# kursawe/OpticalFlow

Hardware: AMD Instinct MI355X
Metric: frame-pairs/sec (higher is better)
Workload: dtype f64; 1 GPU; 1024x1024x256 synthetic translating texture (seed 1), speed_alpha=1, remodelling_alpha=1e4, rtol=1e-06, all 255 pairs solved to the stopping rule; frames_per_gpu=256, pairs_in_flight=255, levels=9, coarse_stencils=float8, vcycle_vectors=coarse_float32, w_cycle_level=1, w_cycle_visits=3, warm_start_stride=3, allgather=False, gather_chunks=1, converged=True

## Files before the change

### opticalflow_amd/csrc/vof.hip

```cpp
#include "vof_device.hpp"
#include "vof_sweep0r.hpp"
#include "vof_sweep0p.hpp"
#include "vof_stream0.hpp"
#include "vof_direct.hpp"
#include "vof_boxflow.hpp"
#include "vof_boxsweep.hpp"
#include "vof_blursweep.hpp"
#include "vof_compare.hpp"
#include "vof_liushen.hpp"
#include "../../include/vof.h"

#include <fcntl.h>
#include <unistd.h>

#include <algorithm>
#include <atomic>
#include <chrono>
#include <cmath>
#include <condition_variable>
#include <cstdio>
#include <cstdlib>
#include <cstring>
#include <mutex>
#include <string>
// ... 60 lines not shown
    int nd = 0;
    int* h_active = nullptr;
    int* h_alist = nullptr;
    PairScalars* h_sc = nullptr;
    double* h_func3 = nullptr;
    char* h_bounce = nullptr;
    hipEvent_t ev_batch[2] = {nullptr, nullptr};
    double* st_movie = nullptr;
    double* st_out[4] = {nullptr, nullptr, nullptr, nullptr};
    double* st_out2[4] = {nullptr, nullptr, nullptr, nullptr};
    hipStream_t copy_stream = nullptr;
    hipEvent_t ev_solved[2] = {nullptr, nullptr}, ev_copied[2] = {nullptr, nullptr}, ev_uploaded[2] = {nullptr, nullptr};
    double* st_movie2 = nullptr;
    double *blur_tmp = nullptr, *blur_w = nullptr, *blur_io = nullptr;
    double* bf_scratch = nullptr;
    double* sw_scratch = nullptr;
    size_t sw_planes = 0;
    bool sw_by_budget = false;
    char* sw_aux = nullptr;
    size_t sw_aux_bytes = 0;
    bool bf_lds_set = false;
    bool bl_lds_set = false;
    bool ls_lds_set = false;
    double* tex_tab = nullptr;
    size_t tex_cap = 0;
    double* gm_V = nullptr;
    GmresState* gm_state = nullptr;
    double* gm_partials = nullptr;
    int* gm_cycle = nullptr;
    int gm_m = 0;
    long long gmres_pairs = 0;
    struct Alloc { void* raw; char* user; size_t bytes; const char* name; int line; };
    std::vector<Alloc> allocs;
    int c_bytes_per_point = 0;
    size_t bytes = 0;
    std::string err;
    const double* frames = nullptr;
    int npairs = 0;
    vof_params prm;
    int cfmt = 0;
    bool fused = true;
    bool fold_stored = false;
    bool fuse_revisit = true;
    bool direct_on = false;
    int dir_cap = 0;
    double *dir_T = nullptr, *dir_tabs = nullptr, *dir_W = nullptr, *dir_r = nullptr, *dir_y = nullptr, *dir_x = nullptr, *dir_t = nullptr;
    int *dir_ipiv = nullptr, *dir_info = nullptr;
    double *dir_R = nullptr, *dir_C = nullptr, *dir_D = nullptr;
    int dir_ld = 0;
    long long direct_pairs = 0;
    bool fuse_rr = true;
    bool fuse_b = true;
    int fused_ends = 3;
    long sweep0r_min_blocks = 512;
    int tail_first = -1;
    size_t tail_lds = 0;
    TailArgs tail;
    int tail_key[6] = {-9, -9, -9, -9, -9, -9};
    bool prof = false;
    int prof_kid = -1, prof_level = -1;
    std::vector<ProfRec> recs;
    std::vector<hipEvent_t> free_events;
    long long prof_dropped = 0;
    double prof_ms[VOF_K_COUNT][16];
    long long prof_n[VOF_K_COUNT][16];
    long long prof_units[VOF_K_COUNT][16];
    double prof_bytes[VOF_K_COUNT][16];
    double prof_moved[VOF_K_COUNT][16];
    int cur_units = 0;
    int dbg_sync = 0;
    long long dbg_seq = 0;
    std::string dbg_fault;
    int dbg_fd = -1;
    bool dbg_canary = false;
    bool dbg_alloc_log = false;
    bool dbg_poison = false;
    size_t part_per_pair = 0;
    vof_ctx* lane_parent = nullptr;
    int lane_lo = 0, lane_slots = 0;
    int dir_ok = -1;
    hipStream_t lane_stream[MAX_LANES] = {};
    hipEvent_t lane_ev[MAX_LANES][2] = {};
    hipEvent_t ev_fork = nullptr;
    hipEvent_t group_ev[MAX_LANES * MAX_LANE_GROUPS] = {};
};

static std::string g_create_error;

namespace {

void dbg_sync_check(vof_ctx* c, const char* what, int level) {
    if (!c->dbg_sync) return;
    ++c->dbg_seq;
    char line[256];
    if (c->dbg_fd >= 0) {
        int n = snprintf(line, sizeof line, "in flight: scope #%lld '%s' level %d, %d pairs, grid %dx%d (%d levels)%-40s\n", c->dbg_seq, what, level,
                         c->cur_units, c->Ni, c->Nj, (int)c->L.size(), "");
        if (pwrite(c->dbg_fd, line, (size_t)n, 0) < 0) {  }
    }
    hipError_t e = hipStreamSynchronize(c->stream);
    hipError_t e2 = hipGetLastError();
    if (e == hipSuccess) e = e2;
    if (e != hipSuccess && c->dbg_fault.empty()) {
        snprintf(line, sizeof line, "VOF_DEBUG_SYNC: scope #%lld, kernel class '%s', level %d, %d pairs, image %dx%d: %s", c->dbg_seq, what, level,
                 c->cur_units, c->Ni, c->Nj, hipGetErrorString(e));
        c->dbg_fault = line;
// ... 602 lines not shown
           s0r_row<2, true, false, 0, float, 1, 0, float>(c, p, f0, nslots, a) || s0r_row<2, true, false, 0, double, 1, 0, float>(c, p, f0, nslots, a) ||
           shapes(IntTag<2>{}, IntTag<0>{}) || shapes(IntTag<2>{}, IntTag<1>{}) || shapes(IntTag<1>{}, IntTag<0>{}) || shapes(IntTag<1>{}, IntTag<1>{});
}

template <int NS, bool EC, bool FZ, int TR, typename ET = double>
bool s0m_row(vof_ctx* c, const L0Pass& p, const Fine0& f0, int nslots, const L0Ptrs& a) {
    if (p.NS != NS || p.EC != EC || p.FROM_ZERO != FZ || p.TRAIL != TR || p.ET32 != is_f32<ET>()) return false;
    k_sweep0m<NS, EC, FZ, TR, ET><<<dim3(p.blocks * nslots), p.block, p.lds, c->stream>>>(
        f0, c->L[0].ni, c->L[0].nj, p.TI, p.PO, p.nx, p.ny, nslots, (const double*)a.x_in, (double*)a.x_out, (const double*)a.b, a.active,
        (const ET*)a.ecoarse, p.nci, p.ncj, a.tr);
    return true;
}
bool launch_s0m(vof_ctx* c, const L0Pass& p, const Fine0& f0, int nslots, const L0Ptrs& a) {
    auto shapes = [&](auto ns) {
        constexpr int NS = decltype(ns)::value;
        return s0m_row<NS, true, false, 1, float>(c, p, f0, nslots, a) || s0m_row<NS, true, false, 0, float>(c, p, f0, nslots, a) ||
               s0m_row<NS, true, false, 1>(c, p, f0, nslots, a) || s0m_row<NS, false, false, 1>(c, p, f0, nslots, a) ||
               s0m_row<NS, true, false, 0>(c, p, f0, nslots, a) || s0m_row<NS, false, true, 0>(c, p, f0, nslots, a) ||
               s0m_row<NS, false, false, 0>(c, p, f0, nslots, a);
    };
    return shapes(IntTag<2>{}) || shapes(IntTag<1>{});
}

template <int NS, bool EC, bool FZ, int PO>
bool s0p_row(vof_ctx* c, const L0Pass& p, const Fine0& f0, int nslots, const L0Ptrs& a) {
    if (p.NS != NS || p.EC != EC || p.FROM_ZERO != FZ || p.PO != PO) return false;
    k_sweep0p<NS, EC, FZ, PO><<<dim3(p.blocks * nslots), p.block, p.lds, c->stream>>>(
        f0, c->L[0].ni, c->L[0].nj, p.TI, p.nx, p.nxp, p.ny, nslots, (const float*)a.x_in, (float*)a.x_out, (const float*)a.b, a.active,
        (const float*)a.ecoarse, p.nci, p.ncj);
    return true;
}
bool launch_s0p(vof_ctx* c, const L0Pass& p, const Fine0& f0, int nslots, const L0Ptrs& a) {
    auto shapes = [&](auto ns, auto po) {
        constexpr int NS = decltype(ns)::value, PO = decltype(po)::value;
        return s0p_row<NS, true, false, PO>(c, p, f0, nslots, a) || s0p_row<NS, false, true, PO>(c, p, f0, nslots, a) ||
               s0p_row<NS, false, false, PO>(c, p, f0, nslots, a);
    };
    return shapes(IntTag<2>{}, IntTag<0>{}) || shapes(IntTag<2>{}, IntTag<1>{}) || shapes(IntTag<1>{}, IntTag<0>{}) || shapes(IntTag<1>{}, IntTag<1>{});
}

template <typename VT, bool EC, bool FZ>
bool s0_row(vof_ctx* c, const L0Pass& p, const Fine0& f0, int nslots, const L0Ptrs& a) {
    if (p.EC != EC || p.FROM_ZERO != FZ) return false;
    k_sweep0<VT, EC, FZ><<<dim3(p.blocks * nslots), p.block, p.lds, c->stream>>>(
        f0, c->L[0].ni, c->L[0].nj, p.TI, p.PO, p.nx, p.ny, nslots, (const VT*)a.x_in, (VT*)a.x_out, (const VT*)a.b, a.active,
        (const VT*)a.ecoarse, p.nci, p.ncj);
    return true;
}
template <typename VT>
bool launch_s0(vof_ctx* c, const L0Pass& p, const Fine0& f0, int nslots, const L0Ptrs& a) {
    return s0_row<VT, true, false>(c, p, f0, nslots, a) || s0_row<VT, false, true>(c, p, f0, nslots, a) || s0_row<VT, false, false>(c, p, f0, nslots, a);
}

void fold_s_epilogue(vof_ctx* c, int np, const L0Pass& p) {
    const size_t len = 3 * c->L[0].npts;
    { Prof pr(c, VOF_K_VECTOR, 0); k_scalar<S_S><<<np, 64, 0, c->stream>>>(c->sc, c->partials, (int)p.blocks, c->active, c->prm.rtol, c->prm.max_iterations); }
    { Prof pr(c, VOF_K_VECTOR, 0);
      if (p.XT32) k_fix_half<float><<<dim3(64, np), RBLK, 0, c->stream>>>(c->kx, (const float*)c->ky, len, c->sc);
      else k_fix_half<double><<<dim3(64, np), RBLK, 0, c->stream>>>(c->kx, (const double*)c->ky, len, c->sc);
      k_clear_half<<<(np + 255) / 256, 256, 0, c->stream>>>(c->sc, np); }
}

template <typename VT>
struct SmoothArgs {
    bool from_zero = false;
    bool reverse = false;
    const VT* ecoarse = nullptr;
    bool ec32 = false;
    bool allow_swap = false;
    bool final_smooth = false;
    bool out64 = false;
    bool skip0 = false;
    void* rr_out = nullptr;
    bool rr_f32 = false;
    int nsweeps = 1;
    bool trail = false;
};

template <typename VT>
void sweep_level_t(vof_ctx* c, int l, const VT* x_in, VT* x_out, const VT* b, int np, ActiveSet active, const SmoothArgs<VT>& a,
                   CycleIO& io) {
    Level& lv = c->L[l];
    const VT* ecoarse = a.ecoarse;
    const int po = a.reverse ? 1 : 0;
    if (l == 0 && lv.C == nullptr) {
        L0Req rq;
        rq.from_zero = x_in == nullptr; rq.po = po; rq.nsweeps = a.nsweeps;
        rq.ec = ecoarse != nullptr; rq.ec32 = a.ec32;
        rq.trail = a.trail && io.trail.v != nullptr; rq.trail_dot = io.trail.dotvec != nullptr;
        rq.rr = a.rr_out != nullptr; rq.rr_f32 = a.rr_f32;
        rq.bf = io.bf_done ? 0 : io.bf_mode;
        rq.x32 = c->h32;
        const L0Pass p = plan_l0_pass<VT>(c, rq);
        if (p.XT32 != c->h32) { c->err = "float32 level-0 hand-off: the planned pass does not store float32"; io.failed = true; return; }
        const S0Trail no_trail{nullptr, nullptr, 0, nullptr};
        const L0Ptrs ptrs{x_in, x_out, b, active, ecoarse,
                          p.rr() ? S0Trail{(double*)a.rr_out, nullptr, 0, nullptr} : (p.trail() ? io.trail : no_trail),
                          p.bf() ? io.bf : S0BSrc{nullptr, nullptr, nullptr, nullptr, nullptr, nullptr}};
        const Fine0 f0{c->frames, frame_stride(c), c->Nj, c->prm.speed_alpha, c->prm.remodelling_alpha, c->prm.reference_quirks, c->pp};
        bool launched = false;
        {
            Prof pr(c, VOF_K_GS0, 0, p.algo, p.moved);
            const int nslots = pair_slots(c, active, np);
            switch (p.fam) {
                case L0_SWEEP0R: launched = launch_s0r(c, p, f0, nslots, ptrs); break;
                case L0_SWEEP0M: launched = launch_s0m(c, p, f0, nslots, ptrs); break;
                case L0_SWEEP0P: launched = launch_s0p(c, p, f0, nslots, ptrs); break;
                case L0_SWEEP0: launched = launch_s0<VT>(c, p, f0, nslots, ptrs); break;
            }
        }
        if (!launched) { c->err = "internal: the library holds no kernel for the planned level-0 pass"; io.failed = true; return; }
        if (p.trail()) io.trail_nblk = (int)p.blocks;
        if (p.rr()) io.rr_done = true;
// ... 540 lines not shown
    for (int p = 0; p < ni; ++p) {
        if (trace && (p < 2 || p == ni - 1)) { HIPCHK(hipStreamSynchronize(s)); fprintf(stderr, "[vof] direct_setup: row %d of %d (m = %d, %d pairs)\n", p, ni, m, np); fflush(stderr); }
        double* Tp = c->dir_T + (size_t)p * ld * ld;
        if (p > 0) k_dir_W<<<gm, 256, 0, s>>>(Tp - (size_t)ld * ld, sT, c->dir_tabs + (size_t)(p - 1) * rowTab, sTab, nj, c->dir_W, sW, ld);
        k_dir_schur<<<gs, 256, 0, s>>>(c->dir_tabs + (size_t)p * rowTab, sTab, nj, p > 0 ? c->dir_W : nullptr, sW, Tp, sT, ld);
        if (blocked) {
            for (int kt = 0; kt < nt; ++kt) {
                k_dir_bgj_panel<<<dim3(nt, 2, np), 256, bgj_lds, s>>>(Tp, sT, ld, kt, c->dir_R, c->dir_C, c->dir_D, c->dir_info);
                k_dir_bgj_update<<<dim3(nt, nt, np), 256, bgj_lds, s>>>(Tp, sT, ld, kt, c->dir_R, c->dir_C, c->dir_D);
            }
        } else {
            k_dir_invert<<<np, 1024, 2 * (size_t)m * sizeof(double), s>>>(Tp, sT, m, c->dir_ipiv, c->dir_info);
        }
    }
    HIPCHK(hipGetLastError());
    std::vector<int> info((size_t)np);
    HIPCHK(hipMemcpyAsync(info.data(), c->dir_info, (size_t)np * sizeof(int), hipMemcpyDeviceToHost, s));
    HIPCHK(hipStreamSynchronize(s));
    for (int k = 0; k < np; ++k)
        if (info[k] != 0) { c->err = "direct preconditioner: a Schur block of pair " + std::to_string(k) + " of the batch is singular"; return -2; }
    return 0;
}

template <typename VT>
int direct_apply_t(vof_ctx* c, VT* z, const VT* r, int np) {
    const int ni = c->L[0].ni, nj = c->L[0].nj, m = 3 * nj, ld = c->dir_ld;
    const size_t sT = (size_t)ni * ld * ld, sTab = (size_t)ni * nj * DIR_TAB, rowTab = (size_t)nj * DIR_TAB, sV = (size_t)ni * m;
    hipStream_t s = c->stream;
    Prof pr(c, VOF_K_COARSE_SOLVE, 0);
    const dim3 gp(64, np), gv((m + 255) / 256, np), gg((m + 63) / 64, np);
    k_dir_permute<const VT, true><<<gp, 256, 0, s>>>(r, c->dir_r, ni, nj);
    for (int p = 0; p < ni; ++p) {
        if (p > 0) k_dir_gemv<<<gg, 256, 0, s>>>(c->dir_T + (size_t)(p - 1) * ld * ld, sT, m, c->dir_y + (size_t)(p - 1) * m, sV, c->dir_t, (size_t)m, ld);
        k_dir_rowupdate<<<gv, 256, 0, s>>>(c->dir_tabs + (size_t)p * rowTab, sTab, nj, -1, c->dir_r + (size_t)p * m, sV,
                                          p > 0 ? c->dir_t : nullptr, (size_t)m, c->dir_y + (size_t)p * m, sV);
    }
    for (int p = ni - 1; p >= 0; --p) {
        k_dir_rowupdate<<<gv, 256, 0, s>>>(c->dir_tabs + (size_t)p * rowTab, sTab, nj, +1, c->dir_y + (size_t)p * m, sV,
                                          p + 1 < ni ? c->dir_x + (size_t)(p + 1) * m : nullptr, sV, c->dir_t, (size_t)m);
        k_dir_gemv<<<gg, 256, 0, s>>>(c->dir_T + (size_t)p * ld * ld, sT, m, c->dir_t, (size_t)m, c->dir_x + (size_t)p * m, sV, ld);
    }
    k_dir_permute<VT, false><<<gp, 256, 0, s>>>(z, c->dir_x, ni, nj);
    return 0;
}

struct BatchReq {
    const double* frames;
    int np;
    const PairParam* table;
    const int* guess;
    bool direct;
    double *vx, *vy, *gm, *speed;
    vof_pair_stats* stats;
};

int solve_batch(vof_ctx* c, const BatchReq& rq) {
    const vof_params& P = c->prm;
    const double* const frames_dev = rq.frames;
    const int np = rq.np;
    vof_pair_stats* const stats = rq.stats;
    struct ReqGuard { vof_ctx* c; ~ReqGuard() { c->pp = nullptr; c->direct_on = false; } } req_guard{c};
    const int* guess_src = nullptr;
    if (rq.table || rq.guess) {
        if (rq.table && !c->pp_buf) { if (int rc = dev_alloc(c, &c->pp_buf, (size_t)c->B)) return rc; }
        if (rq.guess && !c->warm_src) { if (int rc = dev_alloc(c, &c->warm_src, (size_t)c->B)) return rc; }
        HIPCHK(hipStreamSynchronize(c->stream));
        if (rq.table) {
            HIPCHK(hipMemcpyAsync(c->pp_buf, rq.table, (size_t)np * sizeof(PairParam), hipMemcpyHostToDevice, c->stream));
            c->pp = c->pp_buf;
        }
        if (rq.guess) {
            HIPCHK(hipMemcpyAsync(c->warm_src, rq.guess, (size_t)np * sizeof(int), hipMemcpyHostToDevice, c->stream));
            guess_src = c->warm_src;
        }
    }
    c->direct_on = rq.direct;
    struct MaxItGuard { vof_params& p; int saved; ~MaxItGuard() { p.max_iterations = saved; } } max_it_guard{c->prm, c->prm.max_iterations};
    constexpr int MG_ATTEMPT_CAP = 150;
    if (P.preconditioner == 2 && !c->direct_on && c->L.size() > 1 && P.max_iterations > MG_ATTEMPT_CAP && 3 * c->L[0].nj <= 3100 &&
        direct_ok_for_fallback(c))
        c->prm.max_iterations = MG_ATTEMPT_CAP;
    if (stats) HIPCHK(hipEventRecord(c->ev_batch[0], c->stream));
    c->vfloat = (P.vcycle_precision == 1 || P.vcycle_precision == 2) && c->fused && c->L.size() > 1 && !c->direct_on;
    c->vcoarse32 = P.vcycle_precision == 3 && !c->direct_on;
    c->h32 = false;
    if (c->direct_on) {
        if (np > c->dir_cap) { c->err = "batch larger than the direct preconditioner's buffers"; return -1; }
        c->frames = frames_dev;
        c->npairs = np;
        c->cur_units = np;
        if (int rc = direct_setup(c, np)) return rc;
        c->direct_pairs += np;
    } else if (int rc = setup_batch(c, frames_dev, np)) return rc;
    Level& f = c->L[0];
    const size_t len = 3 * f.npts;
    hipStream_t s = c->stream;
    double sx = P.delta_t / P.delta_x;
    const bool zero_guess = !guess_src && (P.initial_v_x == 0.0 && P.initial_v_y == 0.0 && P.initial_remodelling == 0.0);
    double* rh = c->krh;
    const bool fuse_pro = (c->fused_ends & 1) && !zero_guess && residual_copy_ok(c) && !c->direct_on;
    int nbb = c->nblk;
    int nb0 = c->nblk;
    const double* part_r0 = c->partials;
    if (fuse_pro) {
        c->cur_units = np;
        nbb = nb0 = fused_prologue(c, guess_src, P.initial_v_x * sx, P.initial_v_y * sx, P.initial_remodelling, np);
        part_r0 = c->partials + nb0;
    } else {
        Prof p(c, VOF_K_RHS, 0);
        k_rhs_norm<<<rgrid(c, np), RBLK, 0, s>>>(frames_dev, frame_stride(c), c->Nj, f.ni, f.nj, c->kb, zero_guess ? c->kr : nullptr,
                                                c->partials, c->pp);
    }
    { Prof p(c, VOF_K_VECTOR, 0); k_scalar<S_BNORM><<<np, 64, 0, s>>>(c->sc, c->partials, nbb, c->active, P.rtol, P.max_iterations); }
    if (zero_guess) {
        HIPCHK(hipMemsetAsync(c->kx, 0, (size_t)np * len * sizeof(double), s));
        rh = c->kb;
    } else if (!fuse_pro) {
        if (guess_src) {
            Prof p(c, VOF_K_VECTOR, 0, 16.0 * len);
            k_gather_guess<<<rgrid(c, np), RBLK, 0, s>>>(c->kx, c->warm_x, guess_src, len, f.npts, P.initial_v_x * sx, P.initial_v_y * sx,
                                                        P.initial_remodelling);
        } else {
            Prof p(c, VOF_K_VECTOR, 0); k_fill<<<dim3(c->nblk, np), 256, 0, s>>>(c->kx, f.npts, P.initial_v_x * sx, P.initial_v_y * sx, P.initial_remodelling);
        }
        const bool two = residual_copy_ok(c);
        nb0 = residual_d(c, c->kx, c->kb, c->kr, np, ALL_PAIRS, 1, two ? c->krh : nullptr);
        if (!two) HIPCHK(hipMemcpyAsync(c->krh, c->kr, (size_t)np * len * sizeof(double), hipMemcpyDeviceToDevice, s));
        if (!nb0) {
            Prof p(c, VOF_K_REDUCE, 0); k_dot2<<<rgrid(c, np), RBLK, 0, s>>>(c->kr, c->kr, nullptr, nullptr, len, c->partials, ALL_PAIRS);
            nb0 = c->nblk;
        }
    }
    { Prof p(c, VOF_K_VECTOR, 0); k_scalar<S_R0><<<np, 64, 0, s>>>(c->sc, part_r0, nb0, c->active, P.rtol, P.max_iterations); }

    const int bicg_limit = P.krylov_method == 1 ? 0 : (P.krylov_method == 2 ? std::min(P.max_iterations, P.fallback_after) : P.max_iterations);
    int it_total = 0;
    auto bicg_loop = [&](int limit) -> int {
    bool ran_on_r = false;
    for (int it = 0; it < limit; ++it, ++it_total) {
        HIPCHK(hipMemcpyAsync(c->h_active, c->active, np * sizeof(int), hipMemcpyDeviceToHost, s));
        HIPCHK(hipStreamSynchronize(s));
        int nact = 0;
        for (int k = 0; k < np; ++k) nact += c->h_active[k] != 0;
        if (nact == 0) break;
        if (int rc = post_active_list(c, np)) return rc;
        if (it_total == AUTO_F64_AFTER) { if (P.vcycle_precision == 2) c->vfloat = false; c->vcoarse32 = false; }
        c->cur_units = nact;
        c->h32 = handoff32_ok(c);
        const ActiveSet act = listed(c, c->active);
        void* vrhs_p = c->vfloat ? (void*)c->b32 : (void*)c->kp;
        void* vrhs_s = c->vfloat ? (void*)c->b32 : (void*)c->kr;
        const double vsz = (c->vfloat || c->h32) ? 4.0 : 8.0;
        const bool on_r = it == 0 && !c->vfloat;
        const bool fold_b = fold_b_usable(c);
        auto cycle_ok = [c](const CycleIO& io, const char* which) {
            if (io.failed) c->h32 = false;
            else if (io.bf_mode && !io.bf_done) c->err = std::string("folded vector update (") + which + "): not consumed by the cycle";
            else return true;
            return false;
        };
        CycleIO io_p, io_s;
        if (on_r) vrhs_p = (void*)c->kr;
        else if (fold_b && it > 0) {
            const double* p_old = (it == 1 && ran_on_r) ? rh : c->kp;
            io_p.bf = S0BSrc{c->kr, c->kv, p_old, c->kt, c->sc, nullptr};
            io_p.bf_mode = 2;
            std::swap(c->kp, c->kt);
            vrhs_p = (void*)c->kp;
        } else {
            Prof p(c, VOF_K_VECTOR, 0, 8.0 * len * (it == 0 ? 2 : 4) + (c->vfloat ? 4.0 * len : 0.0));
            const double* p_old = (it == 1 && ran_on_r) ? rh : c->kp;
            VDISPATCH(c, (k_update_p<VT><<<rgrid(c, np, act), RBLK, 0, s>>>(c->kp, p_old, c->kr, c->kv, len, c->sc, act,
                                                                     c->vfloat ? (VT*)c->b32 : (VT*)nullptr, it == 0 ? 1 : 0)));
        }
        if (it == 0) ran_on_r = on_r;
        io_p.trail = S0Trail{c->kv, rh, 0, c->partials};
        vcycle(c, &c->ky, vrhs_p, np, act, io_p);
        if (!cycle_ok(io_p, "p")) return -1;
        int nb1 = io_p.trail_nblk ? io_p.trail_nblk : krylov_apply(c, c->ky, c->kv, np, act, rh, 0);
        if (!nb1) { Prof p(c, VOF_K_REDUCE, 0, 16.0 * len); k_dot2<<<rgrid(c, np, act), RBLK, 0, s>>>(rh, c->kv, nullptr, nullptr, len, c->partials, act); nb1 = c->nblk; }
        { Prof p(c, VOF_K_VECTOR, 0); k_scalar<S_ALPHA><<<np, 64, 0, s>>>(c->sc, c->partials, nb1, c->active, P.rtol, P.max_iterations); }
        if (fold_b) {
            io_s.bf = S0BSrc{c->kr, c->kv, nullptr, c->kt, c->sc, c->partials};
            io_s.bf_mode = 1;
            std::swap(c->kr, c->kt);
            vrhs_s = (void*)c->kr;
        } else {
        { Prof p(c, VOF_K_VECTOR, 0, 8.0 * len * 3 + (c->vfloat ? 4.0 * len : 0.0));
          VDISPATCH(c, (k_update_s<VT><<<rgrid(c, np, act), RBLK, 0, s>>>(c->kr, c->kv, len, c->sc, c->partials, act, c->vfloat ? (VT*)c->b32 : (VT*)nullptr))); }
        { Prof p(c, VOF_K_VECTOR, 0); k_scalar<S_S><<<np, 64, 0, s>>>(c->sc, c->partials, c->nblk, c->active, P.rtol, P.max_iterations); }
        { Prof p(c, VOF_K_VECTOR, 0);
          YDISPATCH(c, (k_fix_half<VT><<<dim3(64, np), RBLK, 0, s>>>(c->kx, (const VT*)c->ky, len, c->sc)));
          k_clear_half<<<(np + 255) / 256, 256, 0, s>>>(c->sc, np); }
        }
        io_s.trail = S0Trail{c->kt, c->kr, 1, c->partials};
        vcycle(c, &c->kz, vrhs_s, np, act, io_s);
        if (!cycle_ok(io_s, "s")) return -1;
        int nb2 = io_s.trail_nblk ? io_s.trail_nblk : krylov_apply(c, c->kz, c->kt, np, act, c->kr, 1);
        if (!nb2) { Prof p(c, VOF_K_REDUCE, 0, 16.0 * len); k_dot2<<<rgrid(c, np, act), RBLK, 0, s>>>(c->kt, c->kr, c->kt, c->kt, len, c->partials, act); nb2 = c->nblk; }
        { Prof p(c, VOF_K_VECTOR, 0); k_scalar<S_OMEGA><<<np, 64, 0, s>>>(c->sc, c->partials, nb2, c->active, P.rtol, P.max_iterations); }
        { Prof p(c, VOF_K_VECTOR, 0, 8.0 * len * 6 + 2.0 * vsz * len);
          YDISPATCH(c, (k_update_xr<VT><<<rgrid(c, np, act), RBLK, 0, s>>>(c->kx, (const VT*)c->ky, (const VT*)c->kz, c->kr, c->kt, rh, len, c->sc, c->partials, act))); }
        { Prof p(c, VOF_K_VECTOR, 0); k_scalar<S_R><<<np, 64, 0, s>>>(c->sc, c->partials, c->nblk, c->active, P.rtol, P.max_iterations); }
    }
    c->h32 = false;
    return 0;
    };
    if (int rc = bicg_loop(bicg_limit)) return rc;
    auto independent_residual = [&](bool keep) -> int {
        c->cur_units = np;
        int nb3 = keep ? 0 : residual_d(c, c->kx, c->kb, nullptr, np, ALL_PAIRS, 1);
        if (!nb3) nb3 = residual_d(c, c->kx, c->kb, c->kt, np, ALL_PAIRS, 1);
        if (!nb3) { Prof p(c, VOF_K_REDUCE, 0); k_dot2<<<rgrid(c, np), RBLK, 0, s>>>(c->kt, c->kt, nullptr, nullptr, len, c->partials, ALL_PAIRS); nb3 = c->nblk; }
        { Prof p(c, VOF_K_VECTOR, 0); k_scalar<S_FINAL><<<np, 64, 0, s>>>(c->sc, c->partials, nb3, c->active, P.rtol, P.max_iterations); }
        HIPCHK(hipGetLastError());
        return 0;
    };
    bool finalized = false;
    if ((c->fused_ends & 2) && residual_copy_ok(c)) {
        c->cur_units = np;
        double* fpart = c->partials + (size_t)np * 3 * apply_grid(c, np).nblk;
        const int nb3 = fused_epilogue(c, rq.vx, rq.vy, rq.gm, rq.speed, fpart, np);
        { Prof p(c, VOF_K_VECTOR, 0); k_scalar<S_FINAL><<<np, 64, 0, s>>>(c->sc, c->partials, nb3, c->active, P.rtol, P.max_iterations); }
        { Prof p(c, VOF_K_FINALIZE, 0); k_sum3<<<np, 64, 0, s>>>(fpart, nb3, c->func3); }
        HIPCHK(hipGetLastError());
        finalized = true;
    } else if (int rc = independent_residual(false)) return rc;
    if (bicg_limit > 0) {
        for (int round = 0; round < 3; ++round) {
            { Prof p(c, VOF_K_VECTOR, 0); k_bicg_restart<<<(np + 63) / 64, 64, 0, s>>>(c->sc, c->active, np, P.max_iterations); }
            int nact = count_active(c, np);
            if (nact < 0) { c->err = "stream synchronize failed"; return -2; }
            if (nact == 0) break;
            finalized = false;
            if (int rc = independent_residual(true)) return rc;
            c->cur_units = nact;
            rh = c->krh;
            { Prof p(c, VOF_K_VECTOR, 0, 8.0 * len * 3);
              const ActiveSet act = listed(c, c->active);
              k_restart_vectors<<<rgrid(c, np, act), RBLK, 0, s>>>(c->kr, rh, c->kt, len, act); }
            if (int rc = bicg_loop(std::min(bicg_limit, 8))) return rc;
            if (int rc = independent_residual(false)) return rc;
        }
    }
    if (P.krylov_method != 0) {
        int handed_over = 0;
        if (int rc = gmres_phase(c, np, &handed_over)) return rc;
        if (handed_over) {
            finalized = false;
            if (int rc = independent_residual(false)) return rc;
        }
    }
    if (!finalized) {
        Prof p(c, VOF_K_FINALIZE, 0);
        k_finalize_functionals<<<rgrid(c, np), RBLK, 0, s>>>(frames_dev, frame_stride(c), f.ni, f.nj, P.speed_alpha, P.remodelling_alpha,
                                                             P.reference_quirks, c->kx, P.delta_x / P.delta_t, rq.vx, rq.vy, rq.gm, rq.speed,
                                                             c->partials, c->pp);
        k_sum3<<<np, 64, 0, s>>>(c->partials, c->nblk, c->func3);
    }
    HIPCHK(hipGetLastError());
    if (stats) {
// ... 146 lines not shown
    if (c->h_active) hipHostFree(c->h_active);
    if (c->h_alist) hipHostFree(c->h_alist);
    if (c->h_sc) hipHostFree(c->h_sc);
    if (c->h_func3) hipHostFree(c->h_func3);
    if (c->h_bounce) hipHostFree(c->h_bounce);
    for (int i = 0; i < 2; ++i) if (c->ev_batch[i]) hipEventDestroy(c->ev_batch[i]);
    for (int i = 0; i < 2; ++i) {
        if (c->ev_solved[i]) hipEventDestroy(c->ev_solved[i]);
        if (c->ev_copied[i]) hipEventDestroy(c->ev_copied[i]);
        if (c->ev_uploaded[i]) hipEventDestroy(c->ev_uploaded[i]);
    }
    if (c->copy_stream) hipStreamDestroy(c->copy_stream);
    for (int i = 0; i < MAX_LANES; ++i) {
        if (c->lane_stream[i]) hipStreamDestroy(c->lane_stream[i]);
        for (int j = 0; j < 2; ++j) if (c->lane_ev[i][j]) hipEventDestroy(c->lane_ev[i][j]);
    }
    if (c->ev_fork) hipEventDestroy(c->ev_fork);
    for (hipEvent_t e : c->group_ev) if (e) hipEventDestroy(e);
    if (c->own_stream && c->stream) hipStreamDestroy(c->stream);
    delete c;
}

static int create_impl(vof_ctx* c, int device_id, int n_i, int n_j, int B, void* stream) {
    if (n_i < 4 || n_j < 4) { c->err = "image must be at least 4x4 (the mirror boundary rows need N >= 4)"; return -1; }
    if (B < 1) { c->err = "max_pairs_in_flight must be >= 1"; return -1; }
    int ndev = 0;
    HIPCHK(hipGetDeviceCount(&ndev));
    if (device_id < 0 || device_id >= ndev) { c->err = "no such HIP device"; return -1; }
    HIPCHK(hipSetDevice(device_id));
    c->device = device_id;
    c->Ni = n_i; c->Nj = n_j; c->B = B;
    if (stream) { c->stream = (hipStream_t)stream; c->own_stream = false; }
    else { HIPCHK(hipStreamCreate(&c->stream)); c->own_stream = true; }
    memset(c->prof_ms, 0, sizeof c->prof_ms);
    memset(c->prof_n, 0, sizeof c->prof_n);
    memset(c->prof_units, 0, sizeof c->prof_units);
    memset(c->prof_bytes, 0, sizeof c->prof_bytes);
    memset(c->prof_moved, 0, sizeof c->prof_moved);
    vof_default_params(&c->prm, sizeof c->prm);
    if (const char* e = getenv("VOF_DEBUG_SYNC")) c->dbg_sync = atoi(e);
    if (const char* e = getenv("VOF_DEBUG_CANARY")) c->dbg_canary = e[0] != '0';
    if (const char* e = getenv("VOF_DEBUG_ALLOC_LOG")) c->dbg_alloc_log = e[0] != '0';
    if (const char* e = getenv("VOF_DEBUG_POISON")) c->dbg_poison = e[0] != '0';
    if (c->dbg_sync)
        if (const char* e = getenv("VOF_DEBUG_SYNC_FILE")) c->dbg_fd = open(e, O_WRONLY | O_CREAT, 0644);
    if (const char* e = getenv("VOF_FOLD_STORED")) c->fold_stored = e[0] != '0';
    if (const char* e = getenv("VOF_FUSE_REVISIT")) c->fuse_revisit = e[0] != '0';
    if (const char* e = getenv("VOF_L0_HANDOFF")) c->l0_handoff = e[0] != '0';
    if (const char* e = getenv("VOF_SWEEP0R_MIN_BLOCKS")) c->sweep0r_min_blocks = atol(e);
    if (const char* e = getenv("VOF_ACTIVE_LIST")) c->use_alist = e[0] != '0';
    if (const char* e = getenv("VOF_FUSE_B")) c->fuse_b = e[0] != '0';
    if (const char* e = getenv("VOF_FUSE_RR")) c->fuse_rr = e[0] != '0';
    if (const char* e = getenv("VOF_FUSED_ENDS")) { const int v = atoi(e); if (v >= 0 && v <= 3) c->fused_ends = v; }
    Level l0; l0.ni = n_i - 2; l0.nj = n_j - 2; l0.npts = (size_t)l0.ni * l0.nj;
    c->L.push_back(l0);
    while (std::max(c->L.back().ni, c->L.back().nj) > COARSEST_MAX) {
        Level k; k.ni = (c->L.back().ni + 1) / 2; k.nj = (c->L.back().nj + 1) / 2; k.npts = (size_t)k.ni * k.nj;
        c->L.push_back(k);
    }
    int nl = (int)c->L.size();
    if (nl > 16) { c->err = "too many levels"; return -1; }
    size_t len0 = 3 * l0.npts;
    for (double** v : {&c->kx, &c->kb, &c->kr, &c->krh, &c->kp, &c->kv, &c->kt, &c->ky, &c->kz})
        if (int rc = dev_alloc(c, v, (size_t)B * len0)) return rc;
    for (int l = 0; l < nl; ++l) {
        Level& lv = c->L[l];
        auto valloc = [&](void** q) { double* t = nullptr; int rc = dev_alloc(c, &t, (size_t)B * 3 * lv.npts); *q = t; return rc; };
        if (l + 1 < nl && l > 0) if (int rc = valloc(&lv.r)) return rc;
        if (l + 1 < nl) if (int rc = valloc(&lv.x2)) return rc;
        if (l > 0) {
            if (int rc = valloc(&lv.x)) return rc;
            if (int rc = valloc(&lv.b)) return rc;
        }
        if (nl == 1) {
            double* C = nullptr;
            if (int rc = dev_alloc(c, &C, (size_t)B * 81 * CLay(lv.ni, lv.nj).plane)) return rc;
            lv.C = C;
        }
    }
    if (int rc = ensure_stencil_storage(c, vof_params_default_coarse_precision())) return rc;
    c->nd = 3 * (int)c->L.back().npts;
    {
        int first = -1;
        for (int l = 1; l < nl; ++l) {
            const CLay lay(c->L[l].ni, c->L[l].nj);
            if (c->L[l].npts <= (size_t)TAIL_MAX_PTS && lay.sub <= (size_t)TAIL_MAX_SUB) { first = l; break; }
        }
        if (first >= 0) first = std::max(first, nl - TAIL_MAX_LEVELS);
        if (first >= 1 && first < nl - 1) {
            memset(&c->tail, 0, sizeof c->tail);
            int off = 0;
            for (int l = first; l < nl; ++l) {
                TailLevel& t = c->tail.L[l - first];
                const CLay lay(c->L[l].ni, c->L[l].nj);
                t.ni = c->L[l].ni; t.nj = c->L[l].nj; t.hj = lay.hj; t.sub = (int)lay.sub; t.plane = lay.plane;
                t.xo = off; off += 3 * (t.ni + 2) * (t.nj + 2);
                t.bo = off; off += 3 * t.ni * t.nj;
            }
            c->tail.ro = off; off += 3 * (int)c->L[first].npts;
            c->tail.nl = nl - first;
            c->tail.nd = c->nd;
            c->tail.n_ops = 0;
            c->tail_lds = (size_t)off * sizeof(double);
            if (c->tail_lds <= (size_t)150 * 1024) {
                c->tail_first = first;
                const int lds = (int)c->tail_lds;
// ... 204 lines not shown
        if (P > B && rest <= B && rest > 48) np = rest - std::max(16, rest / 4);
        batches.push_back({k0, np});
        k0 += np;
    }
    return batches;
}

inline size_t next_page(uintptr_t base, size_t offset) { return (size_t)(((base + offset + 4095) & ~(uintptr_t)4095) - base); }

size_t plan_movie_split(uintptr_t base, size_t movie_bytes, size_t first_batch_bytes, bool one_batch) {
    return one_batch ? movie_bytes : std::min(movie_bytes, next_page(base, first_batch_bytes));
}

struct HostRegion { char* ptr; size_t bytes; };
std::vector<HostRegion> plan_output_regions(double* const* outs, const std::vector<HostBatch>& batches, size_t frame_bytes, size_t out_bytes) {
    const size_t nb = batches.size();
    std::vector<HostRegion> regions(nb * 4, HostRegion{nullptr, 0});
    for (int i = 0; i < 4; ++i) {
        if (!outs[i]) continue;
        size_t prev = 0;
        for (size_t bi = 0; bi < nb; ++bi) {
            const size_t end = bi + 1 < nb ? std::min(out_bytes, next_page((uintptr_t)outs[i], (size_t)batches[bi + 1].k0 * frame_bytes)) : out_bytes;
            regions[bi * 4 + i] = HostRegion{(char*)outs[i] + prev, end - prev};
            prev = end;
        }
    }
    return regions;
}

}

extern "C" {

static int two_phase_part(vof_ctx* c, const double* movie, const std::vector<int>& list, size_t a, size_t b, bool phase2, int stride,
                          GroupSync& sync, double* v_x, double* v_y, double* remodelling, double* speed, vof_pair_stats* stats) {
    const vof_params prm = c->prm;
    const size_t len = 3 * c->L[0].npts;
    const int cap = batch_slots(c);
    const int n1 = (int)sync.usable.size();
    std::vector<PairParam> hp((size_t)cap);
    std::vector<int> hsrc((size_t)cap);
    std::vector<vof_pair_stats> st((size_t)cap);
    for (size_t o = a; o < b; o += (size_t)cap) {
        const int np = (int)std::min<size_t>((size_t)cap, b - o);
        {
            std::lock_guard<std::mutex> lk(sync.m);
            for (int i = 0; i < np; ++i) {
                const int k = list[o + i];
                hp[i] = PairParam{prm.speed_alpha, prm.remodelling_alpha, k, k};
                const int src = std::min((k + stride / 2) / stride, n1 - 1);
                hsrc[i] = phase2 && sync.usable[src] ? src : -1;
            }
        }
        if (int rc = solve_batch(c, BatchReq{movie, np, hp.data(), phase2 ? hsrc.data() : nullptr, false, v_x, v_y, remodelling, speed, st.data()}))
            return rc;
        if (!phase2) {
            HIPCHK(hipMemcpyAsync(c->warm_x + o * len, c->kx, (size_t)np * len * sizeof(double), hipMemcpyDeviceToDevice, c->stream));
            std::lock_guard<std::mutex> lk(sync.m);
            for (int i = 0; i < np; ++i) sync.usable[o + i] = st[i].converged && std::isfinite(st[i].relative_residual);
        }
        if (stats)
            for (int i = 0; i < np; ++i) stats[list[o + i]] = st[i];
    }
    return 0;
}

static int two_phase_lane(vof_ctx* c, int lane, const std::vector<LaneGroup>& groups, hipEvent_t* ev, GroupSync& sync, const double* movie,
                          const std::vector<int>& first, const std::vector<int>& rest, int stride, double* v_x, double* v_y,
                          double* remodelling, double* speed, vof_pair_stats* stats) {
    const int ng = (int)groups.size();
    auto publish = [&](int g, bool ok) {
        {
            std::lock_guard<std::mutex> lk(sync.m);
            if (sync.state[g]) return;
            if (!ok) for (int o = groups[g].lo; o < groups[g].hi; ++o) sync.usable[o] = 0;
            sync.state[g] = ok ? 1 : -1;
        }
        sync.cv.notify_all();
    };
    auto run_group = [&](int g) -> int {
        const LaneGroup& G = groups[g];
        if (int rc = two_phase_part(c, movie, first, (size_t)G.lo, (size_t)G.hi, false, stride, sync, v_x, v_y, remodelling, speed, stats)) return rc;
        HIPCHK(hipEventRecord(ev[g], c->stream));
        publish(g, true);
        if (g + 1 < ng) {
            int state;
            {
                std::unique_lock<std::mutex> lk(sync.m);
                if (!sync.cv.wait_for(lk, std::chrono::seconds(60), [&] { return sync.state[g + 1] != 0; })) {
                    c->err = "timed out waiting for the phase-1 solutions of the next pair group";
                    return -2;
                }
                state = sync.state[g + 1];
            }
            if (state > 0) HIPCHK(hipStreamWaitEvent(c->stream, ev[g + 1], 0));
        }
        const size_t ra = (size_t)(std::lower_bound(rest.begin(), rest.end(), G.lo * stride) - rest.begin());
        const size_t rb = g + 1 < ng ? (size_t)(std::lower_bound(rest.begin(), rest.end(), G.hi * stride) - rest.begin()) : rest.size();
        return two_phase_part(c, movie, rest, ra, rb, true, stride, sync, v_x, v_y, remodelling, speed, stats);
    };
    int rc = 0;
    for (int g = ng - 1; g >= 0 && !rc; --g)
        if (groups[g].lane == lane) rc = run_group(g);
    for (int g = 0; g < ng; ++g)
        if (groups[g].lane == lane) publish(g, false);
    return rc;
}

static int solve_stack_two_phase(vof_ctx* c, const double* movie, int P, double* v_x, double* v_y, double* remodelling,
                                 double* speed, vof_pair_stats* stats, int stride, int lanes) {
// ... 1773 lines not shown
```

### opticalflow_amd/csrc/vof_device.hpp

```cpp
#pragma once
#include <hip/hip_runtime.h>
#include <stdint.h>
#include <type_traits>

namespace vof {

constexpr int BX = 64;
constexpr int BY = 4;
constexpr int NT = BX * BY;

struct PairScalars {
    double rho, alpha, omega, beta;
    double bnorm2, rnorm2;
    double tol2;
    int iterations;
    int converged;
    int breakdown;
    int halfstep;
};

struct PairParam {
    double alpha, beta;
    int frame;
    int out;
// ... 1076 lines not shown
        for (size_t i = (size_t)blockIdx.x * RBLK + threadIdx.x; i < len / 2; i += (size_t)gridDim.x * RBLK) {
            double2 a = ldnt2(r2 + i);
            if (!first) {
                const double2 pp = ldnt2(q2 + i), vv = ldnt2(v2 + i);
                a.x = fma(beta, fma(-omega, vv.x, pp.x), a.x);
                a.y = fma(beta, fma(-omega, vv.y, pp.y), a.y);
            }
            stnt2(p2 + i, a);
            if (c2) { V2 t; t.x = (VT)a.x; t.y = (VT)a.y; stnt2(c2 + i, t); }
        }
        return;
    }
    for (size_t i = (size_t)blockIdx.x * RBLK + threadIdx.x; i < len; i += (size_t)gridDim.x * RBLK) {
        double t = r[off + i];
        if (!first) t = fma(beta, fma(-omega, v[off + i], p_old[off + i]), t);
        p[off + i] = t;
        if (pcopy) pcopy[off + i] = (VT)t;
    }
}

template <typename VT>
__global__ __launch_bounds__(RBLK) void k_update_s(double* __restrict__ r, const double* __restrict__ v, size_t len,
                                                   const PairScalars* __restrict__ sc, double* __restrict__ partials,
                                                   const ActiveSet act, VT* __restrict__ scopy) {
    int pair = act.pair(blockIdx.y);
    if (!act.on(pair)) return;
    double alpha = sc[pair].alpha;
    size_t off = (size_t)pair * len;
    double ss = 0;
    if ((len & 1) == 0) {
        typedef typename Vec2<VT>::type V2;
        double2* r2 = reinterpret_cast<double2*>(r + off);
        const double2* v2 = reinterpret_cast<const double2*>(v + off);
        V2* c2 = scopy ? reinterpret_cast<V2*>(scopy + off) : nullptr;
        for (size_t i = (size_t)blockIdx.x * RBLK + threadIdx.x; i < len / 2; i += (size_t)gridDim.x * RBLK) {
            double2 a = ldnt2(r2 + i), vv = ldnt2(v2 + i);
            a.x = fma(-alpha, vv.x, a.x);
            a.y = fma(-alpha, vv.y, a.y);
            stnt2(r2 + i, a);
            if (c2) { V2 t; t.x = (VT)a.x; t.y = (VT)a.y; stnt2(c2 + i, t); }
            ss += a.x * a.x + a.y * a.y;
        }
    } else {
        for (size_t i = (size_t)blockIdx.x * RBLK + threadIdx.x; i < len; i += (size_t)gridDim.x * RBLK) {
            double s = fma(-alpha, v[off + i], r[off + i]);
            r[off + i] = s;
            if (scopy) scopy[off + i] = (VT)s;
            ss += s * s;
        }
    }
    block_store_partials(ss, 0.0, 0.0, partials, 1, gridDim.x, pair, blockIdx.x);
}

template <typename VT>
__global__ __launch_bounds__(RBLK) void k_update_xr(double* __restrict__ x, const VT* __restrict__ y,
                                                    const VT* __restrict__ z, double* __restrict__ r,
                                                    const double* __restrict__ t, const double* __restrict__ rh,
                                                    size_t len, const PairScalars* __restrict__ sc,
                                                    double* __restrict__ partials, const ActiveSet act) {
    int pair = act.pair(blockIdx.y);
    if (!act.on(pair)) return;
    double alpha = sc[pair].alpha, omega = sc[pair].omega;
    size_t off = (size_t)pair * len;
    double rr = 0, rho = 0;
    if ((len & 1) == 0) {
        typedef typename Vec2<VT>::type V2;
        double2* x2 = reinterpret_cast<double2*>(x + off);
        double2* r2 = reinterpret_cast<double2*>(r + off);
        const double2* t2 = reinterpret_cast<const double2*>(t + off);
        const double2* h2 = reinterpret_cast<const double2*>(rh + off);
        const V2* y2 = reinterpret_cast<const V2*>(y + off);
        const V2* z2 = reinterpret_cast<const V2*>(z + off);
        for (size_t i = (size_t)blockIdx.x * RBLK + threadIdx.x; i < len / 2; i += (size_t)gridDim.x * RBLK) {
            double2 xx = ldnt2(x2 + i), a = ldnt2(r2 + i), tt = ldnt2(t2 + i), hh = ldnt2(h2 + i);
            V2 yy = ldnt2(y2 + i), zz = ldnt2(z2 + i);
            xx.x += alpha * (double)yy.x + omega * (double)zz.x;
            xx.y += alpha * (double)yy.y + omega * (double)zz.y;
            stnt2(x2 + i, xx);
            a.x -= omega * tt.x;
            a.y -= omega * tt.y;
            stnt2(r2 + i, a);
            rr += a.x * a.x + a.y * a.y;
            rho += hh.x * a.x + hh.y * a.y;
        }
    } else {
        for (size_t i = (size_t)blockIdx.x * RBLK + threadIdx.x; i < len; i += (size_t)gridDim.x * RBLK) {
            x[off + i] += alpha * (double)y[off + i] + omega * (double)z[off + i];
            double s = r[off + i] - omega * t[off + i];
            r[off + i] = s;
            rr += s * s;
            rho += rh[off + i] * s;
        }
    }
    block_store_partials(rr, rho, 0.0, partials, 2, gridDim.x, pair, blockIdx.x);
}

template <typename VT>
__global__ __launch_bounds__(RBLK) void k_fix_half(double* __restrict__ x, const VT* __restrict__ y, size_t len,
                                                   PairScalars* __restrict__ sc) {
    int pair = blockIdx.y;
    if (sc[pair].halfstep != 1) return;
    double alpha = sc[pair].alpha;
    size_t off = (size_t)pair * len;
    for (size_t i = (size_t)blockIdx.x * RBLK + threadIdx.x; i < len; i += (size_t)gridDim.x * RBLK)
        x[off + i] += alpha * (double)y[off + i];
}
__global__ void k_clear_half(PairScalars* __restrict__ sc, int np) {
    int k = blockIdx.x * blockDim.x + threadIdx.x;
    if (k < np && sc[k].halfstep == 1) sc[k].halfstep = 2;
}

__global__ void k_fill(double* __restrict__ x, size_t npts, double c0, double c1, double c2) {
    int pair = blockIdx.y;
    size_t len = 3 * npts, off = (size_t)pair * len;
    for (size_t i = (size_t)blockIdx.x * blockDim.x + threadIdx.x; i < len; i += (size_t)gridDim.x * blockDim.x)
        x[off + i] = i < npts ? c0 : (i < 2 * npts ? c1 : c2);
}

template <typename TA, typename TB>
__global__ void k_convert(const TA* __restrict__ a, TB* __restrict__ b, size_t n) {
    for (size_t i = (size_t)blockIdx.x * blockDim.x + threadIdx.x; i < n; i += (size_t)gridDim.x * blockDim.x)
        b[i] = (TB)a[i];
}

enum ScalarStep { S_BNORM = 0, S_R0, S_ALPHA, S_S, S_OMEGA, S_R, S_FINAL };

__device__ __forceinline__ double sum_partials(const double* __restrict__ pp, int nblk) {
    double s = 0;
    for (int i = threadIdx.x; i < nblk; i += 64) s += pp[i];
    return wave_sum(s);
}

template <int STEP>
__global__ void k_scalar(PairScalars* __restrict__ sc, const double* __restrict__ partials, int nblk,
                         int* __restrict__ active, double rtol, int max_it) {
    int pair = blockIdx.x;
    if (STEP != S_BNORM && STEP != S_FINAL && !active[pair]) return;
    const double* pp = partials + (size_t)pair * 3 * nblk;
    double a = sum_partials(pp, nblk);
    double b = (STEP == S_OMEGA || STEP == S_R) ? sum_partials(pp + nblk, nblk) : 0.0;
    if (threadIdx.x != 0) return;
    PairScalars& s = sc[pair];
    if (STEP == S_BNORM) {
        s.bnorm2 = a;
        s.tol2 = rtol * rtol * a;
        s.rho = s.alpha = s.omega = 1.0;
        s.beta = 0.0;
        s.iterations = 0;
        s.converged = 0;
        s.breakdown = 0;
        s.halfstep = 0;
        active[pair] = 1;
    } else if (STEP == S_R0) {
        s.rnorm2 = a;
        if (a <= s.tol2) { s.converged = 1; active[pair] = 0; }
        if (max_it <= 0) active[pair] = 0;
        s.beta = a;
        s.rho = a;
// ... 2089 lines not shown
```

Before: 1470 frame-pairs/s.

## Skip zero-fill of x and initial residual copy; solve directly into warm buffer

For zero initial guesses the solver no longer memsets x up front. The first x update and half-step kernels treat x as zero and write it fresh, and a fallback memset covers pairs that never reach an update. The initial residual is read straight from b instead of being written to r, and phase-1 batches solve in place inside the warm-start buffer, which removes a device-to-device copy per batch. These cut full-length passes over f64 vectors, in exchange for more state tracking (x_unset, r0_in_b) and a risk of stale x for inactive pairs.

```diff
diff --git a/opticalflow_amd/csrc/vof.hip b/opticalflow_amd/csrc/vof.hip
--- a/opticalflow_amd/csrc/vof.hip
+++ b/opticalflow_amd/csrc/vof.hip
@@ -136,6 +136,8 @@
     bool fuse_rr = true;
     bool fuse_b = true;
     int fused_ends = 3;
+    int lean_start = 7;
+    bool x_unset = false;
     long sweep0r_min_blocks = 512;
     int tail_first = -1;
     size_t tail_lds = 0;
@@ -844,13 +846,18 @@
     return s0_row<VT, true, false>(c, p, f0, nslots, a) || s0_row<VT, false, true>(c, p, f0, nslots, a) || s0_row<VT, false, false>(c, p, f0, nslots, a);
 }
 
+template <typename VT>
+void fix_half(vof_ctx* c, int np) {
+    const size_t len = 3 * c->L[0].npts;
+    if (c->x_unset) k_fix_half<VT, true><<<dim3(64, np), RBLK, 0, c->stream>>>(c->kx, (const VT*)c->ky, len, c->sc, c->active);
+    else k_fix_half<VT><<<dim3(64, np), RBLK, 0, c->stream>>>(c->kx, (const VT*)c->ky, len, c->sc);
+    k_clear_half<<<(np + 255) / 256, 256, 0, c->stream>>>(c->sc, np);
+}
 void fold_s_epilogue(vof_ctx* c, int np, const L0Pass& p) {
-    const size_t len = 3 * c->L[0].npts;
     { Prof pr(c, VOF_K_VECTOR, 0); k_scalar<S_S><<<np, 64, 0, c->stream>>>(c->sc, c->partials, (int)p.blocks, c->active, c->prm.rtol, c->prm.max_iterations); }
     { Prof pr(c, VOF_K_VECTOR, 0);
-      if (p.XT32) k_fix_half<float><<<dim3(64, np), RBLK, 0, c->stream>>>(c->kx, (const float*)c->ky, len, c->sc);
-      else k_fix_half<double><<<dim3(64, np), RBLK, 0, c->stream>>>(c->kx, (const double*)c->ky, len, c->sc);
-      k_clear_half<<<(np + 255) / 256, 256, 0, c->stream>>>(c->sc, np); }
+      if (p.XT32) fix_half<float>(c, np);
+      else fix_half<double>(c, np); }
 }
 
 template <typename VT>
@@ -1497,6 +1504,7 @@
     bool direct;
     double *vx, *vy, *gm, *speed;
     vof_pair_stats* stats;
+    double* x_home = nullptr;
 };
 
 int solve_batch(vof_ctx* c, const BatchReq& rq) {
@@ -1504,7 +1512,8 @@
     const double* const frames_dev = rq.frames;
     const int np = rq.np;
     vof_pair_stats* const stats = rq.stats;
-    struct ReqGuard { vof_ctx* c; ~ReqGuard() { c->pp = nullptr; c->direct_on = false; } } req_guard{c};
+    struct ReqGuard { vof_ctx* c; double* kx; ~ReqGuard() { c->pp = nullptr; c->direct_on = false; c->kx = kx; c->x_unset = false; } } req_guard{c, c->kx};
+    if (rq.x_home) c->kx = rq.x_home;
     const int* guess_src = nullptr;
     if (rq.table || rq.guess) {
         if (rq.table && !c->pp_buf) { if (int rc = dev_alloc(c, &c->pp_buf, (size_t)c->B)) return rc; }
@@ -1544,6 +1553,10 @@
     const bool zero_guess = !guess_src && (P.initial_v_x == 0.0 && P.initial_v_y == 0.0 && P.initial_remodelling == 0.0);
     double* rh = c->krh;
     const bool fuse_pro = (c->fused_ends & 1) && !zero_guess && residual_copy_ok(c) && !c->direct_on;
+    const int bicg_limit = P.krylov_method == 1 ? 0 : (P.krylov_method == 2 ? std::min(P.max_iterations, P.fallback_after) : P.max_iterations);
+    const bool lean = zero_guess && bicg_limit > 0 && !c->direct_on;
+    c->x_unset = lean && (c->lean_start & 1);
+    bool r0_in_b = lean && (c->lean_start & 2) && !c->vfloat && fold_b_usable(c);
     int nbb = c->nblk;
     int nb0 = c->nblk;
     const double* part_r0 = c->partials;
@@ -1553,12 +1566,18 @@
         part_r0 = c->partials + nb0;
     } else {
         Prof p(c, VOF_K_RHS, 0);
-        k_rhs_norm<<<rgrid(c, np), RBLK, 0, s>>>(frames_dev, frame_stride(c), c->Nj, f.ni, f.nj, c->kb, zero_guess ? c->kr : nullptr,
+        k_rhs_norm<<<rgrid(c, np), RBLK, 0, s>>>(frames_dev, frame_stride(c), c->Nj, f.ni, f.nj, c->kb, zero_guess && !r0_in_b ? c->kr : nullptr,
                                                 c->partials, c->pp);
     }
     { Prof p(c, VOF_K_VECTOR, 0); k_scalar<S_BNORM><<<np, 64, 0, s>>>(c->sc, c->partials, nbb, c->active, P.rtol, P.max_iterations); }
+    auto zero_x = [&]() -> int {
+        Prof p(c, VOF_K_VECTOR, 0, 8.0 * len);
+        HIPCHK(hipMemsetAsync(c->kx, 0, (size_t)np * len * sizeof(double), s));
+        c->x_unset = false;
+        return 0;
+    };
     if (zero_guess) {
-        HIPCHK(hipMemsetAsync(c->kx, 0, (size_t)np * len * sizeof(double), s));
+        if (!c->x_unset) { if (int rc = zero_x()) return rc; }
         rh = c->kb;
     } else if (!fuse_pro) {
         if (guess_src) {
@@ -1578,7 +1597,6 @@
     }
     { Prof p(c, VOF_K_VECTOR, 0); k_scalar<S_R0><<<np, 64, 0, s>>>(c->sc, part_r0, nb0, c->active, P.rtol, P.max_iterations); }
 
-    const int bicg_limit = P.krylov_method == 1 ? 0 : (P.krylov_method == 2 ? std::min(P.max_iterations, P.fallback_after) : P.max_iterations);
     int it_total = 0;
     auto bicg_loop = [&](int limit) -> int {
     bool ran_on_r = false;
@@ -1587,7 +1605,10 @@
         HIPCHK(hipStreamSynchronize(s));
         int nact = 0;
         for (int k = 0; k < np; ++k) nact += c->h_active[k] != 0;
-        if (nact == 0) break;
+        if (nact == 0) {
+            if (c->x_unset) { c->cur_units = np; if (int rc = zero_x()) return rc; }
+            break;
+        }
         if (int rc = post_active_list(c, np)) return rc;
         if (it_total == AUTO_F64_AFTER) { if (P.vcycle_precision == 2) c->vfloat = false; c->vcoarse32 = false; }
         c->cur_units = nact;
@@ -1605,7 +1626,14 @@
             return false;
         };
         CycleIO io_p, io_s;
-        if (on_r) vrhs_p = (void*)c->kr;
+        const double* r_in = c->kr;
+        if (r0_in_b) {
+            if (on_r && fold_b) r_in = c->kb;
+            else { Prof p(c, VOF_K_VECTOR, 0, 16.0 * len);
+                   HIPCHK(hipMemcpyAsync(c->kr, c->kb, (size_t)np * len * sizeof(double), hipMemcpyDeviceToDevice, s)); }
+            r0_in_b = false;
+        }
+        if (on_r) vrhs_p = (void*)r_in;
         else if (fold_b && it > 0) {
             const double* p_old = (it == 1 && ran_on_r) ? rh : c->kp;
             io_p.bf = S0BSrc{c->kr, c->kv, p_old, c->kt, c->sc, nullptr};
@@ -1626,7 +1654,7 @@
         if (!nb1) { Prof p(c, VOF_K_REDUCE, 0, 16.0 * len); k_dot2<<<rgrid(c, np, act), RBLK, 0, s>>>(rh, c->kv, nullptr, nullptr, len, c->partials, act); nb1 = c->nblk; }
         { Prof p(c, VOF_K_VECTOR, 0); k_scalar<S_ALPHA><<<np, 64, 0, s>>>(c->sc, c->partials, nb1, c->active, P.rtol, P.max_iterations); }
         if (fold_b) {
-            io_s.bf = S0BSrc{c->kr, c->kv, nullptr, c->kt, c->sc, c->partials};
+            io_s.bf = S0BSrc{r_in, c->kv, nullptr, c->kt, c->sc, c->partials};
             io_s.bf_mode = 1;
             std::swap(c->kr, c->kt);
             vrhs_s = (void*)c->kr;
@@ -1635,8 +1663,7 @@
           VDISPATCH(c, (k_update_s<VT><<<rgrid(c, np, act), RBLK, 0, s>>>(c->kr, c->kv, len, c->sc, c->partials, act, c->vfloat ? (VT*)c->b32 : (VT*)nullptr))); }
         { Prof p(c, VOF_K_VECTOR, 0); k_scalar<S_S><<<np, 64, 0, s>>>(c->sc, c->partials, c->nblk, c->active, P.rtol, P.max_iterations); }
         { Prof p(c, VOF_K_VECTOR, 0);
-          YDISPATCH(c, (k_fix_half<VT><<<dim3(64, np), RBLK, 0, s>>>(c->kx, (const VT*)c->ky, len, c->sc)));
-          k_clear_half<<<(np + 255) / 256, 256, 0, s>>>(c->sc, np); }
+          YDISPATCH(c, fix_half<VT>(c, np)); }
         }
         io_s.trail = S0Trail{c->kt, c->kr, 1, c->partials};
         vcycle(c, &c->kz, vrhs_s, np, act, io_s);
@@ -1644,14 +1671,18 @@
         int nb2 = io_s.trail_nblk ? io_s.trail_nblk : krylov_apply(c, c->kz, c->kt, np, act, c->kr, 1);
         if (!nb2) { Prof p(c, VOF_K_REDUCE, 0, 16.0 * len); k_dot2<<<rgrid(c, np, act), RBLK, 0, s>>>(c->kt, c->kr, c->kt, c->kt, len, c->partials, act); nb2 = c->nblk; }
         { Prof p(c, VOF_K_VECTOR, 0); k_scalar<S_OMEGA><<<np, 64, 0, s>>>(c->sc, c->partials, nb2, c->active, P.rtol, P.max_iterations); }
-        { Prof p(c, VOF_K_VECTOR, 0, 8.0 * len * 6 + 2.0 * vsz * len);
-          YDISPATCH(c, (k_update_xr<VT><<<rgrid(c, np, act), RBLK, 0, s>>>(c->kx, (const VT*)c->ky, (const VT*)c->kz, c->kr, c->kt, rh, len, c->sc, c->partials, act))); }
+        { Prof p(c, VOF_K_VECTOR, 0, 8.0 * len * (c->x_unset ? 5 : 6) + 2.0 * vsz * len);
+          if (c->x_unset) YDISPATCH(c, (k_update_xr<VT, true><<<rgrid(c, np, act), RBLK, 0, s>>>(c->kx, (const VT*)c->ky, (const VT*)c->kz, c->kr, c->kt, rh, len, c->sc, c->partials, act)));
+          else YDISPATCH(c, (k_update_xr<VT><<<rgrid(c, np, act), RBLK, 0, s>>>(c->kx, (const VT*)c->ky, (const VT*)c->kz, c->kr, c->kt, rh, len, c->sc, c->partials, act)));
+          c->x_unset = false; }
         { Prof p(c, VOF_K_VECTOR, 0); k_scalar<S_R><<<np, 64, 0, s>>>(c->sc, c->partials, c->nblk, c->active, P.rtol, P.max_iterations); }
     }
     c->h32 = false;
     return 0;
     };
     if (int rc = bicg_loop(bicg_limit)) return rc;
+    r0_in_b = false;
+    if (c->x_unset) { c->cur_units = np; if (int rc = zero_x()) return rc; }
     auto independent_residual = [&](bool keep) -> int {
         c->cur_units = np;
         int nb3 = keep ? 0 : residual_d(c, c->kx, c->kb, nullptr, np, ALL_PAIRS, 1);
@@ -1904,6 +1935,7 @@
     if (const char* e = getenv("VOF_FUSE_B")) c->fuse_b = e[0] != '0';
     if (const char* e = getenv("VOF_FUSE_RR")) c->fuse_rr = e[0] != '0';
     if (const char* e = getenv("VOF_FUSED_ENDS")) { const int v = atoi(e); if (v >= 0 && v <= 3) c->fused_ends = v; }
+    if (const char* e = getenv("VOF_LEAN_START")) { const int v = atoi(e); if (v >= 0 && v <= 7) c->lean_start = v; }
     Level l0; l0.ni = n_i - 2; l0.nj = n_j - 2; l0.npts = (size_t)l0.ni * l0.nj;
     c->L.push_back(l0);
     while (std::max(c->L.back().ni, c->L.back().nj) > COARSEST_MAX) {
@@ -2214,10 +2246,13 @@
                 hsrc[i] = phase2 && sync.usable[src] ? src : -1;
             }
         }
-        if (int rc = solve_batch(c, BatchReq{movie, np, hp.data(), phase2 ? hsrc.data() : nullptr, false, v_x, v_y, remodelling, speed, st.data()}))
+        const bool at_home = !phase2 && (c->lean_start & 4);
+        if (int rc = solve_batch(c, BatchReq{movie, np, hp.data(), phase2 ? hsrc.data() : nullptr, false, v_x, v_y, remodelling, speed, st.data(),
+                                             at_home ? c->warm_x + o * len : nullptr}))
             return rc;
         if (!phase2) {
-            HIPCHK(hipMemcpyAsync(c->warm_x + o * len, c->kx, (size_t)np * len * sizeof(double), hipMemcpyDeviceToDevice, c->stream));
+            if (!at_home)
+                HIPCHK(hipMemcpyAsync(c->warm_x + o * len, c->kx, (size_t)np * len * sizeof(double), hipMemcpyDeviceToDevice, c->stream));
             std::lock_guard<std::mutex> lk(sync.m);
             for (int i = 0; i < np; ++i) sync.usable[o + i] = st[i].converged && std::isfinite(st[i].relative_residual);
         }
diff --git a/opticalflow_amd/csrc/vof_device.hpp b/opticalflow_amd/csrc/vof_device.hpp
--- a/opticalflow_amd/csrc/vof_device.hpp
+++ b/opticalflow_amd/csrc/vof_device.hpp
@@ -1152,7 +1152,7 @@
     block_store_partials(ss, 0.0, 0.0, partials, 1, gridDim.x, pair, blockIdx.x);
 }
 
-template <typename VT>
+template <typename VT, bool X0 = false>
 __global__ __launch_bounds__(RBLK) void k_update_xr(double* __restrict__ x, const VT* __restrict__ y,
                                                     const VT* __restrict__ z, double* __restrict__ r,
                                                     const double* __restrict__ t, const double* __restrict__ rh,
@@ -1172,10 +1172,10 @@
         const V2* y2 = reinterpret_cast<const V2*>(y + off);
         const V2* z2 = reinterpret_cast<const V2*>(z + off);
         for (size_t i = (size_t)blockIdx.x * RBLK + threadIdx.x; i < len / 2; i += (size_t)gridDim.x * RBLK) {
-            double2 xx = ldnt2(x2 + i), a = ldnt2(r2 + i), tt = ldnt2(t2 + i), hh = ldnt2(h2 + i);
+            double2 xx = X0 ? double2{0.0, 0.0} : ldnt2(x2 + i), a = ldnt2(r2 + i), tt = ldnt2(t2 + i), hh = ldnt2(h2 + i);
             V2 yy = ldnt2(y2 + i), zz = ldnt2(z2 + i);
-            xx.x += alpha * (double)yy.x + omega * (double)zz.x;
-            xx.y += alpha * (double)yy.y + omega * (double)zz.y;
+            xx.x += fma(alpha, (double)yy.x, omega * (double)zz.x);
+            xx.y += fma(alpha, (double)yy.y, omega * (double)zz.y);
             stnt2(x2 + i, xx);
             a.x -= omega * tt.x;
             a.y -= omega * tt.y;
@@ -1185,7 +1185,9 @@
         }
     } else {
         for (size_t i = (size_t)blockIdx.x * RBLK + threadIdx.x; i < len; i += (size_t)gridDim.x * RBLK) {
-            x[off + i] += alpha * (double)y[off + i] + omega * (double)z[off + i];
+            double xx = X0 ? 0.0 : x[off + i];
+            xx += fma(alpha, (double)y[off + i], omega * (double)z[off + i]);
+            x[off + i] = xx;
             double s = r[off + i] - omega * t[off + i];
             r[off + i] = s;
             rr += s * s;
@@ -1195,15 +1197,22 @@
     block_store_partials(rr, rho, 0.0, partials, 2, gridDim.x, pair, blockIdx.x);
 }
 
-template <typename VT>
+template <typename VT, bool X0 = false>
 __global__ __launch_bounds__(RBLK) void k_fix_half(double* __restrict__ x, const VT* __restrict__ y, size_t len,
-                                                   PairScalars* __restrict__ sc) {
+                                                   PairScalars* __restrict__ sc, const int* __restrict__ active = nullptr) {
     int pair = blockIdx.y;
-    if (sc[pair].halfstep != 1) return;
+    size_t off = (size_t)pair * len;
+    if (sc[pair].halfstep != 1) {
+        if (X0 && !active[pair])
+            for (size_t i = (size_t)blockIdx.x * RBLK + threadIdx.x; i < len; i += (size_t)gridDim.x * RBLK) x[off + i] = 0.0;
+        return;
+    }
     double alpha = sc[pair].alpha;
-    size_t off = (size_t)pair * len;
-    for (size_t i = (size_t)blockIdx.x * RBLK + threadIdx.x; i < len; i += (size_t)gridDim.x * RBLK)
-        x[off + i] += alpha * (double)y[off + i];
+    for (size_t i = (size_t)blockIdx.x * RBLK + threadIdx.x; i < len; i += (size_t)gridDim.x * RBLK) {
+        double xx = X0 ? 0.0 : x[off + i];
+        xx = fma(alpha, (double)y[off + i], xx);
+        x[off + i] = xx;
+    }
 }
 __global__ void k_clear_half(PairScalars* __restrict__ sc, int np) {
     int k = blockIdx.x * blockDim.x + threadIdx.x;
```

Result: no change. 1476 frame-pairs/s, median of 4 (+0.4%).
